# ComparativeGenomicsToolkit/cactus

Hardware: NVIDIA H100
Metric: BAR POA DP Gcells/sec and ends/sec at 1/2/4/8 H100 vs reference CPU BAR (higher is better)
Workload: dtype int32

## Files before the change

cactus_b200/csrc/poa_cta.cuh:

```cuda
#pragma once
#include <cuda_runtime.h>
#include "poa_graph.cuh"
#include "graph_phases.cuh"

namespace barb200 {

__device__ __forceinline__ bool grow_in_par(Graph &g, int t) {
    if (g.in_n[t] < g.in_cap[t]) return true;
    const int ncap = g.in_cap[t] ? g.in_cap[t] * 2 : 2;
    const int noff = atomicAdd(&g.in_used, ncap);
    if (noff + ncap > g.in_pool) { g.err = JOB_ERR_EDGE_CAP; return false; }
    for (int i = 0; i < g.in_n[t]; ++i) { g.in_id[noff + i] = g.in_id[g.in_off[t] + i]; g.in_w[noff + i] = g.in_w[g.in_off[t] + i]; }
    g.in_off[t] = noff; g.in_cap[t] = ncap;
    return true;
}
__device__ __forceinline__ bool grow_out_par(Graph &g, int f) {
    if (g.out_n[f] < g.out_cap[f]) return true;
    const int ncap = g.out_cap[f] ? g.out_cap[f] * 2 : 2;
    const int noff = atomicAdd(&g.out_used, ncap);
    if (noff + ncap > g.out_pool) { g.err = JOB_ERR_EDGE_CAP; return false; }
    const int W = g.W;
    for (int i = 0; i < g.out_n[f]; ++i) {
        g.out_id[noff + i] = g.out_id[g.out_off[f] + i]; g.out_w[noff + i] = g.out_w[g.out_off[f] + i];
        for (int w = 0; w < W; ++w) g.out_rid[(int64_t)(noff + i) * W + w] = g.out_rid[(int64_t)(g.out_off[f] + i) * W + w];
    }
    for (int i = g.out_n[f]; i < ncap; ++i) for (int w = 0; w < W; ++w) g.out_rid[(int64_t)(noff + i) * W + w] = 0;
    g.out_off[f] = noff; g.out_cap[f] = ncap;
    return true;
}
__device__ __forceinline__ void graph_add_edge_par(Graph &g, int from, int to, int check_edge, int read_id) {
    int out_i = -1;
    if (check_edge) {
        const int io = g.in_off[to], in = g.in_n[to];
        for (int i = 0; i < in; ++i) if (g.in_id[io + i] == from) { g.in_w[io + i] += 1; break; }
        const int oo = g.out_off[from], on = g.out_n[from];
        for (int i = 0; i < on; ++i) if (g.out_id[oo + i] == to) { g.out_w[oo + i] += 1; out_i = i; break; }
    }
    if (out_i < 0) {
        if (!grow_in_par(g, to) || !grow_out_par(g, from)) return;
        const int ip = g.in_off[to] + g.in_n[to]; g.in_id[ip] = from; g.in_w[ip] = 1; g.in_n[to]++;
        out_i = g.out_n[from];
        const int op = g.out_off[from] + out_i; g.out_id[op] = to; g.out_w[op] = 1; g.out_n[from]++;
    }
    g.out_rid[(int64_t)(g.out_off[from] + out_i) * g.W + (read_id >> 6)] |= 1ULL << (read_id & 63);
}

__device__ void cta_add_first_sequence(Graph &g, const uint8_t *seq, int len, int read_id) {
    const int tid = threadIdx.x, T = blockDim.x, W = g.W;
    if (len + 2 > g.node_cap) { if (tid == 0) g.err = JOB_ERR_NODE_CAP; __syncthreads(); return; }
    if (2 * (len + 1) > g.in_pool || 2 * (len + 1) > g.out_pool) { if (tid == 0) g.err = JOB_ERR_EDGE_CAP; __syncthreads(); return; }
    const int rw = read_id >> 6; const uint64_t rb = 1ULL << (read_id & 63);
    for (int i = tid; i <= len; i += T) {
        const int to = i < len ? 2 + i : SINK_ID, from = i == 0 ? SRC_ID : 1 + i;
        g.in_off[to] = 2 * i; g.in_n[to] = 1; g.in_cap[to] = 2; g.in_id[2 * i] = from; g.in_w[2 * i] = 1;
        g.out_off[from] = 2 * i; g.out_n[from] = 1; g.out_cap[from] = 2; g.out_id[2 * i] = to; g.out_w[2 * i] = 1;
        for (int w = 0; w < W; ++w) { g.out_rid[(int64_t)(2 * i) * W + w] = w == rw ? rb : 0; g.out_rid[(int64_t)(2 * i + 1) * W + w] = 0; }
        if (i < len) { g.base[to] = seq[i]; g.aln_n[to] = 0; }
        g.index_to_node[i + 1] = to; g.node_to_index[to] = i + 1;
    }
    if (tid == 0) { g.index_to_node[0] = SRC_ID; g.node_to_index[SRC_ID] = 0; }
    if (tid == 0) { g.node_n = len + 2; g.in_used = 2 * (len + 1); g.out_used = 2 * (len + 1); }
    __syncthreads();
}

__device__ void cta_fuse_alignment(Graph &g, const uint8_t *seq, int L, const uint64_t *cigar, int n_cigar, int read_id, int *ws,
                                   unsigned char *scr, int scr_bytes) {
    const int tid = threadIdx.x, T = blockDim.x;
    if (n_cigar == 0) return;
    int *node_of = g.tmp0, *is_new = g.tmp1;
    for (int c = tid; c < n_cigar; c += T) {
        const uint64_t cg = cigar[c];
        const int op = (int)(cg & 0xf);
        if (op == CMATCH) {
            const int node_id = (int)((cg >> 34) & 0x3fffffff), q = (int)((cg >> 4) & 0x3fffffff);
            const uint8_t b = seq[q];
            if (g.base[node_id] == b) { node_of[q] = node_id; is_new[q] = 0; }
            else {
                const int a = graph_aligned_with_base(g, node_id, b);
                if (a != -1) { node_of[q] = a; is_new[q] = 0; } else { node_of[q] = -1 - node_id; is_new[q] = 1; }
            }
        } else if (op == CINS) {
            const int qe = (int)((cg >> 34) & 0x3fffffff), len = (int)((cg >> 4) & 0x3fffffff);
            for (int q = qe - len + 1; q <= qe; ++q) { node_of[q] = INT32_MIN; is_new[q] = 1; }
        }
    }
    __syncthreads();
    const int first_new = g.node_n;
    const int n_new = cta_excl_scan(is_new, L, ws);
    if (first_new + n_new > g.node_cap) { if (tid == 0) g.err = JOB_ERR_NODE_CAP; __syncthreads(); return; }
    for (int q = tid; q < L; q += T) {
        const int m = node_of[q];
        if (m >= 0) { is_new[q] = 0; continue; }
        const int nid = first_new + is_new[q];
        g.base[nid] = seq[q]; g.aln_n[nid] = 0;
        g.in_off[nid] = 0; g.in_n[nid] = 0; g.in_cap[nid] = 0; g.out_off[nid] = 0; g.out_n[nid] = 0; g.out_cap[nid] = 0;
        if (m != INT32_MIN) graph_add_aligned(g, -1 - m, nid);
        node_of[q] = nid; is_new[q] = 1;
    }
    if (tid == 0) g.node_n = first_new + n_new;
    __syncthreads();
    if (g.err) return;
    if (splice_smem_fits(L, first_new, first_new + n_new, scr_bytes)) splice_order_smem(g, node_of, L, first_new, n_new, scr, ws, T);
    else {
        int *anc = g.remain, *cnt = g.msa_rank, *new_i2n = g.tmp1;
        const int n_old = first_new;
        for (int q = tid; q < L; q += T) {
            const int v = node_of[q];
            int e = v < first_new ? g.node_to_index[v] : -1;
            for (int k = 0; k < g.aln_n[v]; ++k) { const int a = g.aln_id[v * 4 + k]; if (a < first_new) e = max(e, g.node_to_index[a]); }
            anc[q] = e;
        }
        for (int i = tid; i < n_old; i += T) cnt[i] = 0;
        __syncthreads();
        cta_incl_max_scan(anc, L, ws);
        for (int q = tid; q < L; q += T) if (node_of[q] >= first_new) atomicAdd(&cnt[max(anc[q], 0)], 1);
        __syncthreads();
        cta_excl_scan(cnt, n_old, ws);
        for (int i = tid; i < n_old; i += T) new_i2n[i + cnt[i]] = g.index_to_node[i];
        for (int q = tid; q < L; q += T) { const int v = node_of[q]; if (v >= first_new) new_i2n[max(anc[q], 0) + 1 + (v - first_new)] = v; }
        __syncthreads();
        for (int k = tid; k < first_new + n_new; k += T) { const int v = new_i2n[k]; g.index_to_node[k] = v; g.node_to_index[v] = k; }
        __syncthreads();
    }
    for (int q = tid; q <= L; q += T) {
        const int from = q == 0 ? SRC_ID : node_of[q - 1], to = q == L ? SINK_ID : node_of[q];
        const int fresh = (q > 0 && from >= first_new) || (q < L && to >= first_new);
        graph_add_edge_par(g, from, to, fresh ? 0 : 1, read_id);
    }
    __syncthreads();
}


__device__ __forceinline__ void prefetch_l2(const void *p) { asm volatile("prefetch.global.L2 [%0];" ::"l"(p)); }

__device__ int warp_backtrack_step(const RowTables &rt, const DpState &d, const PoaParams &P, const int *smat8, const uint8_t *q,
                                   int &i, int &j, int &cur_op, int &len) {
    const unsigned FULLM = 0xffffffffu;
    const int lane = threadIdx.x & 31, inf = P.inf_min, e1 = P.e1, e2 = P.e2, oe1 = P.o1 + P.e1, oe2 = P.o2 + P.e2;
    len = 1;
    const RowRec rc = rt.rec[i];
    const RowInfo ri = d.info[i];
    const int *rowi = d.planes + d.row_off[i];
    const int npre = rc.base_npre >> 8;
    const int s = smat8[8 * (rc.base_npre & 0xff) + q[j - 1]];
    int hij = inf; unsigned cij = (unsigned)E_NEG16 | (unsigned)E_NEG16 << 16;
    if (j >= ri.beg && j <= ri.end) { hij = __ldcg(rowi + plane_index(ri.beg, ri.end, 0, j)); cij = (unsigned)__ldcg(rowi + plane_index(ri.beg, ri.end, 1, j)); }
    int hk0 = inf;
    if ((cur_op & OP_F) && j - 1 - lane >= ri.beg && j - 1 - lane <= ri.end) hk0 = __ldcg(rowi + plane_index(ri.beg, ri.end, 0, j - 1 - lane));
    int pi = -1, pm = inf, ph = inf, pe1 = inf, pe2 = inf; bool m_in = false, e_in = false;
    auto probe = [&](int kb) {
        const int k = kb + lane;
        pi = -1; m_in = false; e_in = false;
        if (k >= npre) return;
        pi = k == 0 ? rc.pre0 : rt.pre_row[rc.pre_off + k];
        const RowInfo pin = d.info[pi];
        const int *prow = d.planes + d.row_off[pi];
        m_in = (cur_op & OP_M) && j - 1 >= pin.beg && j - 1 <= pin.end;
        e_in = (cur_op & OP_E) && j >= pin.beg && j <= pin.end;
        if (m_in) pm = __ldcg(prow + plane_index(pin.beg, pin.end, 0, j - 1));
        if (e_in) {
            ph = __ldcg(prow + plane_index(pin.beg, pin.end, 0, j));
            const unsigned code = (unsigned)__ldcg(prow + plane_index(pin.beg, pin.end, 1, j));
            pe1 = e_decode(ph, (int)(code & 0xffffu), inf); pe2 = e_decode(ph, (int)(code >> 16), inf);
        }
    };
    if (cur_op & OP_M) {
        for (int kb = 0; kb < npre; kb += 32) {
            probe(kb);
            const unsigned hit = __ballot_sync(FULLM, m_in && pm + s == hij);
            if (hit) { i = __shfl_sync(FULLM, pi, __ffs(hit) - 1); --j; cur_op = OP_ALL; return CMATCH; }
        }
    }
    if (cur_op & OP_E) {
        const int own_e1 = e_decode(hij, (int)(cij & 0xffffu), inf), own_e2 = e_decode(hij, (int)(cij >> 16), inf);
        for (int kb = 0; kb < npre; kb += 32) {
            if (npre > 32 || !(cur_op & OP_M)) probe(kb);
            const bool ok1 = e_in && (cur_op & OP_E1) && ((cur_op & OP_M) ? hij == pe1 : own_e1 == pe1 - e1);
            const bool ok2 = e_in && (cur_op & OP_E2) && ((cur_op & OP_M) ? hij == pe2 : own_e2 == pe2 - e2);
            const unsigned hit = __ballot_sync(FULLM, ok1 || ok2);
            if (hit) {
                const int f = __ffs(hit) - 1;
                const int nop = ok1 ? ((ph - oe1 == pe1) ? (OP_M | OP_F) : OP_E1) : ((ph - oe2 == pe2) ? (OP_M | OP_F) : OP_E2);
                cur_op = __shfl_sync(FULLM, nop, f); i = __shfl_sync(FULLM, pi, f);
                return CDEL;
            }
        }
    }
    if (cur_op & OP_F) {
        if (!(cur_op & OP_M)) return -1;
        const int avail = j - ri.beg;
        int t1_max;
        if (e1 > e2) t1_max = oe2 >= oe1 ? (oe2 - oe1) / (e1 - e2) + 1 : 0;
        else t1_max = (e1 < e2 || oe1 <= oe2) ? avail : 0;
        if (t1_max > avail) t1_max = avail;
        for (int which = 0; which < 2; ++which) {
            if (!(cur_op & (which ? OP_F2 : OP_F1))) continue;
            const int oe = which ? oe2 : oe1, e = which ? e2 : e1, tmax = which ? avail : t1_max;
            for (int t0 = 0; t0 < tmax; t0 += 32) {
                const int t = t0 + lane + 1;
                int hk = hk0;
                if (t0 > 0) { hk = inf; if (t <= avail) hk = __ldcg(rowi + plane_index(ri.beg, ri.end, 0, j - t)); }
                const unsigned hit = __ballot_sync(FULLM, t <= tmax && hk == hij + oe + (t - 1) * e);
                if (hit) { len = __ffs(hit); len += t0; j -= len; cur_op = OP_M | OP_E; return CINS; }
            }
        }
    }
    return -1;
}

__device__ void warp_backtrack(Graph &g, const RowTables &rt, DpState &d, const PoaParams &P, const int *smat8, const uint8_t *q, int L) {
    const unsigned FULLM = 0xffffffffu;
    const int lane = threadIdx.x & 31, inf = P.inf_min;
    if (lane == 0) { dp_best_cell(g, rt, d, P, L); d.fc_row = -1; d.fc_hi = -1; }
    __syncwarp();
    int i = d.best_i, j = d.best_j, cur_op = OP_ALL, nc = 0, last_op = -1;
    uint64_t *cg = d.cigar; const int cap = d.cigar_cap;
    int fail = 0;
    auto push = [&](int op, int len, int node_id, int query_id) {
        if (nc == 0 || op != CINS || last_op != CINS) {
            if (nc >= cap) { fail = JOB_ERR_CIGAR_CAP; return; }
            if (lane == 0) {
                const uint64_t n_id = (uint64_t)(int64_t)node_id, q_id = (uint64_t)(int64_t)query_id, l = (uint64_t)len;
                cg[nc] = op == CMATCH ? (n_id << 34 | q_id << 4 | (uint64_t)op) : op == CINS ? (q_id << 34 | l << 4 | (uint64_t)op) : (n_id << 34 | l << 4 | (uint64_t)op);
            }
            ++nc;
        } else if (lane == 0) cg[nc - 1] += (uint64_t)len << 4;
        last_op = op;
    };
    if (j < L) push(CINS, L - j, -1, L - 1);
#ifdef BT_PROFILE
    long long pf_t0 = clock64(), pf_run_t = 0, pf_step_t = 0; int pf_iters = 0, pf_runs = 0, pf_cells = 0, pf_steps = 0, pf_ins = 0;
#endif
    while (i > 0 && j > 0 && !fail) {
        int run = 0;
#ifdef BT_PROFILE
        long long pf_a = clock64();
#endif
        if (cur_op == OP_ALL) {
            int c = i - lane, pre = -1, base = 0, n_ok = 0, node = 0;
            RowInfo ric; ric.beg = 0; ric.end = -1; ric.left = 0; ric.right = 0;
            int64_t ro = 0;
            bool fresh = true;
#pragma unroll 1
            for (int it = 0; it < 4; ++it) {
                if (fresh) {
                    pre = -1;
                    if (c > 0) { const RowRec rc = rt.rec[c]; base = rc.base_npre & 0xff; pre = (rc.base_npre >> 8) ? rc.pre0 : -1; node = g.index_to_node[c]; }
                    if (c >= 0) { ric = d.info[c]; ro = d.row_off[c]; }
                }
                const int nxt = __shfl_down_sync(FULLM, c, 1);
                const bool ok = lane < 31 && pre >= 0 && pre == nxt;
                n_ok = __ffs(~__ballot_sync(FULLM, ok)) - 1;
                if (n_ok >= 31 || it == 3) break;
                const int pre_b = __shfl_sync(FULLM, pre, n_ok);
                if (pre_b < 0) break;
                fresh = lane > n_ok;
                if (fresh) c = pre_b - (lane - n_ok - 1);
            }
            const int jj = j - lane;
            int hv = inf, inb = 0;
            if (lane <= n_ok && c >= 0 && jj >= 0) {
                inb = jj >= ric.beg && jj <= ric.end;
                if (inb) hv = __ldcg(d.planes + ro + plane_index(ric.beg, ric.end, 0, jj));
            }
            const int cl = c - 32, jl = jj - 32;
            RowInfo ril; ril.beg = 0; ril.end = -1; ril.left = 0; ril.right = 0;
            int64_t rol = 0;
            if (cl >= 0 && jl >= 0) { ril = d.info[cl]; rol = d.row_off[cl]; prefetch_l2(rt.rec + cl); prefetch_l2(g.index_to_node + cl); }
            const int h_next = __shfl_down_sync(FULLM, hv, 1), inb_next = __shfl_down_sync(FULLM, inb, 1);
            bool hit = false;
            if (lane < n_ok && c > 0 && jj >= 1 && inb_next) hit = h_next + smat8[8 * base + q[jj - 1]] == hv;
            run = __ffs(~__ballot_sync(FULLM, hit)) - 1;
            if (run > 0) {
                if (nc + run > cap) fail = JOB_ERR_CIGAR_CAP;
                else {
                    if (lane < run) cg[nc + lane] = (uint64_t)node << 34 | (uint64_t)(jj - 1) << 4 | (uint64_t)CMATCH;
                    nc += run; last_op = CMATCH;
                    i = __shfl_sync(FULLM, c, run); j -= run;
                }
            }
            if (cl >= 0 && jl >= 0 && jl <= ril.end) prefetch_l2(d.planes + rol + plane_index(ril.beg, ril.end, 0, jl < ril.beg ? ril.beg : jl));
        }
#ifdef BT_PROFILE
        long long pf_b = clock64(); if (cur_op == OP_ALL) { pf_run_t += pf_b - pf_a; ++pf_iters; if (run) { ++pf_runs; pf_cells += run; } }
#endif
        if (run == 0 && !fail) {
            const int id = g.index_to_node[i], jq = j - 1;
            int len = 1;
            const int op = warp_backtrack_step(rt, d, P, smat8, q, i, j, cur_op, len);
            if (op < 0) fail = JOB_ERR_BACKTRACK; else push(op, len, id, jq);
#ifdef BT_PROFILE
            pf_step_t += clock64() - pf_b; ++pf_steps; if (op == CINS) ++pf_ins;
#endif
        }
    }
#ifdef BT_PROFILE
    if (lane == 0 && blockIdx.x == 0) printf("bt L=%d total=%lld run_t=%lld step_t=%lld iters=%d runs=%d cells=%d steps=%d ins=%d\n", L, clock64() - pf_t0, pf_run_t, pf_step_t, pf_iters, pf_runs, pf_cells, pf_steps, pf_ins);
#endif
    if (!fail && j > 0) push(CINS, j, -1, j - 1);
    if (fail) { if (lane == 0) g.err = fail; return; }
    if (lane == 0) d.n_cigar = nc;
    __syncwarp();
    for (int a = lane; a < nc >> 1; a += 32) { const uint64_t t = cg[a]; cg[a] = cg[nc - 1 - a]; cg[nc - 1 - a] = t; }
    __syncwarp();
}

struct BfsScratch { uint32_t *optr; uint16_t *odst, *queue, *indeg; uint8_t *alnn; };

__device__ __forceinline__ size_t bfs_scratch_bytes(int n, int E) { return (size_t)4 * (n + 1) + (size_t)2 * E + 4 * (size_t)n + n + 16; }

__device__ void bfs_index_smem(Graph &g, const BfsScratch &B) {
    const int n = g.node_n;
    int head = 0, tail = 0;
    B.queue[tail++] = SRC_ID;
    while (head < tail) {
        const int cur = B.queue[head++];
        if (cur == SINK_ID) {
            if (head != n) g.err = JOB_ERR_TOPO;
            return;
        }
        const uint32_t o0 = B.optr[cur], o1 = B.optr[cur + 1];
        for (uint32_t i = o0; i < o1; ++i) {
            const int o = B.odst[i];
            const int left = (int)B.indeg[o] - 1; B.indeg[o] = (uint16_t)left;
            if (left == 0) {
                const int an = B.alnn[o];
                bool ok = true;
                for (int j = 0; j < an; ++j) if (B.indeg[g.aln_id[o * 4 + j]] != 0) { ok = false; break; }
                if (!ok) continue;
                B.queue[tail++] = (uint16_t)o;
                for (int j = 0; j < an; ++j) B.queue[tail++] = (uint16_t)g.aln_id[o * 4 + j];
            }
        }
    }
    g.err = JOB_ERR_TOPO;
}

__device__ void cta_topo_sort(Graph &g, RowTables &rt, unsigned char *scr, int scr_bytes, int *ws, bool have_order) {
    const int tid = threadIdx.x, T = blockDim.x, n = g.node_n;
    if (have_order && topo_smem_fits(n, scr_bytes)) { topo_rows_smem(g, rt, scr, ws, T); return; }
    if (have_order) {
        for (int v = tid; v < n; v += T) graph_sort_node_edges(g, v);
        __syncthreads();
    } else {
    for (int v = tid; v < n; v += T) g.tmp0[v] = g.out_n[v];
    __syncthreads();
    const int E = cta_excl_scan(g.tmp0, n, ws);
    if (n < 65536 && bfs_scratch_bytes(n, E) <= (size_t)scr_bytes) {
        BfsScratch B;
        B.optr = reinterpret_cast<uint32_t *>(scr);
        B.odst = reinterpret_cast<uint16_t *>(B.optr + n + 1);
        B.queue = B.odst + E; B.indeg = B.queue + n;
        B.alnn = reinterpret_cast<uint8_t *>(B.indeg + n);
        for (int v = tid; v < n; v += T) {
            const uint32_t o = (uint32_t)g.tmp0[v];
            B.optr[v] = o;
            const int oo = g.out_off[v], on = g.out_n[v];
            for (int i = 0; i < on; ++i) B.odst[o + i] = (uint16_t)g.out_id[oo + i];
            B.indeg[v] = (uint16_t)g.in_n[v]; B.alnn[v] = g.aln_n[v];
        }
        if (tid == 0) B.optr[n] = (uint32_t)E;
        __syncthreads();
        if (T > 32) {
            if (tid == 0) bfs_index_smem(g, B);
            else if (tid >= 32) for (int v = tid - 32; v < n; v += T - 32) graph_sort_node_edges(g, v);
        } else {
            if (tid == 0) bfs_index_smem(g, B);
            __syncwarp();
            for (int v = tid; v < n; v += T) graph_sort_node_edges(g, v);
        }
        __syncthreads();
        if (g.err) return;
        for (int k = tid; k < n; k += T) { const int v = B.queue[k]; g.index_to_node[k] = v; g.node_to_index[v] = k; }
    } else {
        if (tid == 0) graph_bfs_index(g);
        __syncthreads();
        if (g.err) return;
        for (int v = tid; v < n; v += T) graph_sort_node_edges(g, v);
    }
    __syncthreads();
    }
    int *nx[2] = {g.tmp0, g.tmp1}, *dd[2] = {g.remain, g.msa_rank};
    for (int v = tid; v < n; v += T) {
        int nxt = SINK_ID, dist = 0;
        if (v != SINK_ID) {
            int max_w = -1;
            const int oo = g.out_off[v], on = g.out_n[v];
            for (int i = 0; i < on; ++i) if (g.out_w[oo + i] > max_w) { max_w = g.out_w[oo + i]; nxt = g.out_id[oo + i]; }
            dist = 1;
        }
        nx[0][v] = nxt; dd[0][v] = dist;
    }
    __syncthreads();
    int cur = 0;
    for (int span = 1; span < n; span <<= 1, cur ^= 1) {
        for (int v = tid; v < n; v += T) {
            const int nv = nx[cur][v];
            dd[cur ^ 1][v] = dd[cur][v] + dd[cur][nv];
            nx[cur ^ 1][v] = nx[cur][nv];
        }
        __syncthreads();
    }
    if (cur == 0) { for (int v = tid; v < n; v += T) g.remain[v] -= 1; }
    else { for (int v = tid; v < n; v += T) g.remain[v] = g.msa_rank[v] - 1; }
    __syncthreads();
    for (int r = tid; r < n; r += T) g.tmp0[r] = g.in_n[g.index_to_node[r]];
    __syncthreads();
    cta_excl_scan(g.tmp0, n, ws);
    for (int r = tid; r < n; r += T) graph_build_row(g, rt, r, g.tmp0[r]);
    __syncthreads();
}


__device__ void cta_msa_rank(Graph &g, unsigned char *scr, int scr_bytes, int *ws, int *msa_len_out) {
    const int tid = threadIdx.x, T = blockDim.x, n = g.node_n;
    for (int v = tid; v < n; v += T) g.tmp0[v] = g.out_n[v];
    __syncthreads();
    const int E = cta_excl_scan(g.tmp0, n, ws);
    if (n < 65535 && bfs_scratch_bytes(n, E) + 2 * (size_t)n <= (size_t)scr_bytes) {
        BfsScratch B;
        B.optr = reinterpret_cast<uint32_t *>(scr);
        B.odst = reinterpret_cast<uint16_t *>(B.optr + n + 1);
        B.queue = B.odst + E; B.indeg = B.queue + n;
        uint16_t *rk = B.indeg + n;
        B.alnn = reinterpret_cast<uint8_t *>(rk + n);
        for (int v = tid; v < n; v += T) {
            const uint32_t o = (uint32_t)g.tmp0[v];
            B.optr[v] = o;
            const int oo = g.out_off[v], on = g.out_n[v];
            for (int i = 0; i < on; ++i) B.odst[o + i] = (uint16_t)g.out_id[oo + i];
            B.indeg[v] = (uint16_t)g.in_n[v]; B.alnn[v] = g.aln_n[v];
        }
        if (tid == 0) B.optr[n] = (uint32_t)E;
        __syncthreads();
        if (tid == 0) {
            uint16_t *st = B.queue;
            int sp = 0, rank = 0, len = -1;
            st[sp++] = SRC_ID; rk[SRC_ID] = 0xffff;
            while (sp > 0) {
                const int cur = st[--sp];
                if (rk[cur] == 0xffff) {
                    rk[cur] = (uint16_t)rank;
                    for (int i = 0; i < B.alnn[cur]; ++i) rk[g.aln_id[cur * 4 + i]] = (uint16_t)rank;
                    ++rank;
                }
                if (cur == SINK_ID) { len = (int)rk[SINK_ID] - 1; break; }
                const uint32_t o0 = B.optr[cur], o1 = B.optr[cur + 1];
                for (uint32_t i = o0; i < o1; ++i) {
                    const int o = B.odst[i];
                    const int left = (int)B.indeg[o] - 1; B.indeg[o] = (uint16_t)left;
                    if (left == 0) {
                        const int an = B.alnn[o];
                        bool ok = true;
                        for (int j = 0; j < an; ++j) if (B.indeg[g.aln_id[o * 4 + j]] != 0) { ok = false; break; }
                        if (!ok) continue;
                        st[sp++] = (uint16_t)o; rk[o] = 0xffff;
                        for (int j = 0; j < an; ++j) { const int a = g.aln_id[o * 4 + j]; st[sp++] = (uint16_t)a; rk[a] = 0xffff; }
                    }
                }
            }
            if (len < 0) g.err = JOB_ERR_TOPO;
            *msa_len_out = len;
        }
        __syncthreads();
        if (g.err) return;
        for (int v = tid; v < n; v += T) g.msa_rank[v] = rk[v];
    } else {
        if (tid == 0) *msa_len_out = graph_msa_rank(g);
    }
    __syncthreads();
}

}
```

cactus_b200/csrc/poa_kernel.cu:

```cuda
#include <cuda_runtime.h>
#include <stdint.h>
#include "poa_graph.cuh"
#include "poa_cta.cuh"
#include "poa_kernel.cuh"

namespace barb200 {

#define FULL 0xffffffffu

struct KShared {
    Graph g; RowTables rt; DpState d;
    int job, msa_len_s, abort_s;
    __align__(256) int smat[5 * 8];
    int wF[2][2][32];
    int wM[2][4][32];
    RowRec rec[2];
    RowInfo ring_info[2];
};

__device__ __forceinline__ int4 ld4cg(const int *p) { return __ldcg(reinterpret_cast<const int4 *>(p)); }
__device__ __forceinline__ void st4(int *p, int a, int b, int c, int d) {
    asm volatile("st.global.v4.s32 [%0], {%1, %2, %3, %4};" ::"l"(p), "r"(a), "r"(b), "r"(c), "r"(d) : "memory");
}
__device__ __forceinline__ void sts4(unsigned a, int x, int y, int z, int w) {
    asm volatile("st.shared.v4.s32 [%0], {%1, %2, %3, %4};" ::"r"(a), "r"(x), "r"(y), "r"(z), "r"(w) : "memory");
}
__device__ __forceinline__ int4 lds4(unsigned a) {
    int4 v;
    asm volatile("ld.shared.v4.s32 {%0, %1, %2, %3}, [%4];" : "=r"(v.x), "=r"(v.y), "=r"(v.z), "=r"(v.w) : "r"(a) : "memory");
    return v;
}
__device__ __forceinline__ int lds1(unsigned a) {
    int v;
    asm volatile("ld.shared.s32 %0, [%1];" : "=r"(v) : "r"(a) : "memory");
    return v;
}
__device__ __forceinline__ int lds_const(unsigned a) {
    int v;
    asm("ld.shared.s32 %0, [%1];" : "=r"(v) : "r"(a));
    return v;
}
__device__ __forceinline__ int max3(int a, int b, int c) { return max(max(a, b), c); }
__device__ __forceinline__ void cp_async16(void *smem, const void *gmem) {
    asm volatile("cp.async.cg.shared.global [%0], [%1], 16;" ::"r"((unsigned)__cvta_generic_to_shared(smem)), "l"(gmem) : "memory");
}
__device__ __forceinline__ void cp_async_wait_all() { asm volatile("cp.async.wait_all;" ::: "memory"); }
__device__ __forceinline__ void store_pad(int *tp, int64_t cs, int NEG) {
#pragma unroll
    for (int c = 0; c < TB / CHUNK; ++c) st4(tp + c * cs, c < CPT / CHUNK ? NEG : 0, c < CPT / CHUNK ? NEG : 0, c < CPT / CHUNK ? NEG : 0, c < CPT / CHUNK ? NEG : 0);
}


template <bool MASKED>
__device__ __forceinline__ void row_pass1(int (&H)[CPT], int (&E1)[CPT], int (&E2)[CPT], unsigned mbase, const uint32_t (&qo)[4],
                                          int j0, int beg, int end, int NEG, int e1, int e2, int &agg1, int &agg2) {
#pragma unroll
    for (int e = 0; e < CPT; ++e) {
        const int s = lds_const(__byte_perm(qo[e >> 2], mbase, 0x7650 | (e & 3)));
        int h = __vimax3_s32(H[e] + s, E1[e], E2[e]);
        if (MASKED) {
            const bool inb = (unsigned)(j0 + e - beg) <= (unsigned)(end - beg);
            h = inb ? h : NEG; E1[e] = inb ? E1[e] : NEG; E2[e] = inb ? E2[e] : NEG;
        }
        H[e] = h;
    }
    int a1 = H[CPT - 1], a2 = H[CPT - 1];
#pragma unroll
    for (int e = CPT - 2; e >= 0; --e) { a1 = __viaddmax_s32(a1, e1, H[e]); a2 = __viaddmax_s32(a2, e2, H[e]); }
    agg1 = max(agg1, a1 + j0 * e1); agg2 = max(agg2, a2 + j0 * e2);
}

template <bool ROW0>
__device__ __forceinline__ void pred_chunk(int (&H)[CPT], int (&E1)[CPT], int (&E2)[CPT], int oc, int4 h4, int4 d4, int NEG) {
    const int h[CHUNK] = {h4.x, h4.y, h4.z, h4.w}, dv[CHUNK] = {d4.x, d4.y, d4.z, d4.w};
#pragma unroll
    for (int u = 0; u < CHUNK; ++u) {
        const int e = oc * CHUNK + u;
        const int c1 = dv[u] & 0xffff, c2 = (int)((unsigned)dv[u] >> 16);
        if (e + 1 < CPT) H[e + 1] = max(H[e + 1], h[u]);
        E1[e] = max(E1[e], ROW0 && c1 == E_NEG16 ? NEG : h[u] - c1); E2[e] = max(E2[e], ROW0 && c2 == E_NEG16 ? NEG : h[u] - c2);
    }
}

template <int MODE, int RING_NT>
__device__ __forceinline__ void row_pass2(int (&H)[CPT], int (&E1)[CPT], int (&E2)[CPT], int F1, int F2, int j0, int beg, int end, int NEG,
                                          int e1, int e2, int oe1, int oe2, int *tp, int64_t cs, unsigned rs, int &tmax) {
#pragma unroll
    for (int oc = 0; oc < CPT / CHUNK; ++oc) {
        int dd[CHUNK];
#pragma unroll
        for (int u = 0; u < CHUNK; ++u) {
            const int e = oc * CHUNK + u, hp = H[e];
            int h = __vimax3_s32(hp, F1, F2);
            F1 = __viaddmax_s32(F1, -e1, hp - oe1); F2 = __viaddmax_s32(F2, -e2, hp - oe2);
            int x1 = __viaddmax_s32(E1[e], -e1, h - oe1);
            int x2 = __viaddmax_s32(E2[e], -e2, h - oe2);
            if (MODE == 1) {
                const bool inb = (unsigned)(j0 + e - beg) <= (unsigned)(end - beg);
                h = inb ? h : NEG; x1 = inb ? x1 : NEG; x2 = inb ? x2 : NEG;
            } else if (MODE == 2) {
                const bool inb = j0 + e <= end;
                h = inb ? h : NEG; x1 = inb ? x1 : NEG; x2 = inb ? x2 : NEG;
            }
            H[e] = h; E1[e] = x1; E2[e] = x2;
            dd[u] = __byte_perm(h - x1, h - x2, 0x5410);
            tmax = max(tmax, h);
        }
        st4(tp + oc * cs, H[oc * CHUNK], H[oc * CHUNK + 1], H[oc * CHUNK + 2], H[oc * CHUNK + 3]);
        st4(tp + (CPT / CHUNK + oc) * cs, dd[0], dd[1], dd[2], dd[3]);
        if (RING_NT) {
            sts4(rs + oc * RING_NT * 16, H[oc * CHUNK], H[oc * CHUNK + 1], H[oc * CHUNK + 2], H[oc * CHUNK + 3]);
            sts4(rs + (CPT / CHUNK + oc) * RING_NT * 16, dd[0], dd[1], dd[2], dd[3]);
        }
    }
}

template <bool MASKED>
__device__ __forceinline__ void row_argmax(const int (&H)[CPT], int v, int j0, int beg, int end, int &tl, int &tr) {
    unsigned m = 0;
#pragma unroll
    for (int e = 0; e < CPT; ++e) m |= H[e] == v ? 1u << e : 0u;
    if (MASKED) {
        const int lo = max(beg - j0, 0), hi = min(end - j0, CPT - 1);
        m &= (2u << hi) - (1u << lo);
    }
    if (m) { tl = j0 + __ffs(m) - 1; tr = j0 + 31 - __clz(m); }
}

template <int NT>
__device__ long long dp_sweep(KShared &S, const BatchArgs &A, const uint8_t *__restrict__ qg, int L, uint4 *qsm, unsigned ring) {
    constexpr int RING_NT = poa_ring_bytes(NT) ? NT : 0;
    constexpr unsigned SLOT = NT * TB * sizeof(int), RCS = NT * 16;
    const int tid = threadIdx.x, lane = tid & 31, warp = tid >> 5, nwarps = NT >> 5;
    const unsigned my_ring = ring + tid * 16;
    const PoaParams &P = A.P;
    uint8_t *const sb = A.slots + (int64_t)blockIdx.x * A.lay.slot_bytes;
    const RowRec *const rec_tab = reinterpret_cast<const RowRec *>(sb + A.lay.o_row_rec);
    const int *const pre_row = reinterpret_cast<const int *>(sb + A.lay.o_pre_row);
    RowInfo *const info = reinterpret_cast<RowInfo *>(sb + A.lay.o_row_info);
    int64_t *const row_off = reinterpret_cast<int64_t *>(sb + A.lay.o_row_off);
    int *const planes = A.planes + (int64_t)blockIdx.x * A.lay.plane_cap;
    const int64_t plane_cap = A.lay.plane_cap;
    const int node_n = S.g.node_n, R = node_n - 1;
    const int NEG = P.inf_min, e1 = P.e1, e2 = P.e2, oe1 = P.o1 + P.e1, oe2 = P.o2 + P.e2;
    const int w = P.wb + (int)(P.wf * L);
    const int pn_shift = reference_lane_count(P, L, node_n) == 16 ? 4 : 3;
    static_assert(CPT == 16, "shifts below assume 16 columns per thread");
    const int j0 = tid * CPT;

    uint32_t qo[4] = {0u, 0u, 0u, 0u};
#pragma unroll
    for (int e = 0; e < CPT; ++e) {
        const int j = j0 + e;
        const uint32_t c = (j >= 1 && j <= L) ? qg[j - 1] : 5u;
        qo[e >> 2] |= (4u * c) << ((e & 3) * 8);
    }
    qsm[tid] = make_uint4(qo[0], qo[1], qo[2], qo[3]);
    const unsigned smat_s = (unsigned)__cvta_generic_to_shared(S.smat);

    int H[CPT], E1[CPT], E2[CPT];
    bool prev_active;
    int prev_beg = 0, prev_end, prev_left = 0, prev_right = 0;
    int cur_blk = 0, cells = 0;

    {
        const int dd = L - rec_tab[0].rd;
        prev_end = min(L, max(0, dd) + w);
        const int nT = prev_end / CPT + 1, nTs = row_blocks(0, prev_end);
        if ((int64_t)nTs * TB > plane_cap) return -1;
        prev_active = tid < nT;
        int D[CPT];
#pragma unroll
        for (int e = 0; e < CPT; ++e) {
            const int j = j0 + e;
            if (j == 0) { H[e] = 0; E1[e] = -oe1; E2[e] = -oe2; D[e] = oe1 | (oe2 << 16); }
            else if (j <= prev_end) { H[e] = max(-P.o1 - e1 * j, -P.o2 - e2 * j); E1[e] = NEG; E2[e] = NEG; D[e] = E_NEG16 | (E_NEG16 << 16); }
            else { H[e] = E1[e] = E2[e] = NEG; D[e] = 0; }
        }
        if (tid < nTs) {
            int *tp = planes + chunk_index(nTs, tid, 0);
            const int64_t cs = chunk_index(nTs, 0, 1);
#pragma unroll
            for (int oc = 0; oc < CPT / CHUNK; ++oc) {
                st4(tp + oc * cs, H[oc * CHUNK], H[oc * CHUNK + 1], H[oc * CHUNK + 2], H[oc * CHUNK + 3]);
                st4(tp + (CPT / CHUNK + oc) * cs, D[oc * CHUNK], D[oc * CHUNK + 1], D[oc * CHUNK + 2], D[oc * CHUNK + 3]);
            }
        }
        if (RING_NT) {
#pragma unroll
            for (int oc = 0; oc < CPT / CHUNK; ++oc) {
                sts4(my_ring + oc * RCS, H[oc * CHUNK], H[oc * CHUNK + 1], H[oc * CHUNK + 2], H[oc * CHUNK + 3]);
                sts4(my_ring + (CPT / CHUNK + oc) * RCS, D[oc * CHUNK], D[oc * CHUNK + 1], D[oc * CHUNK + 2], D[oc * CHUNK + 3]);
            }
        }
        if (lane == 31) S.wM[0][3][warp] = H[CPT - 1];
        if (tid == 0) {
            RowInfo ri; ri.beg = 0; ri.end = prev_end; ri.left = 0; ri.right = 0; info[0] = ri; row_off[0] = 0;
            if (RING_NT) S.ring_info[0] = ri;
        }
        cur_blk = nTs; cells = prev_end + 1;
        if (tid == 0) { cp_async16(&S.rec[1], rec_tab + (R > 1 ? 1 : 0)); cp_async_wait_all(); }
    }
    __syncthreads();

    for (int r = 1; r < R; ++r) {
        const int par = r & 1;
        const RowRec rec = S.rec[par];
        if (tid == 0 && r + 1 < R) cp_async16(&S.rec[par ^ 1], rec_tab + r + 1);
        const int b = rec.base_npre & 0xff, npre = rec.base_npre >> 8;
        const int dd = L - rec.rd;
        int maxL = node_n, maxR = 0, min_pre_beg = 0x7fffffff;
        bool has_prev = false;
        if (npre == 1 && rec.pre0 == r - 1) {
            maxL = min(node_n, prev_left + 1); maxR = prev_right + 1; min_pre_beg = prev_beg; has_prev = true;
        } else {
#pragma unroll 1
            for (int k = 0; k < npre; ++k) {
                const int p = k == 0 ? rec.pre0 : pre_row[rec.pre_off + k];
                int pl, pr, pb;
                if (p == r - 1) { pl = prev_left; pr = prev_right; pb = prev_beg; has_prev = true; }
                else if (RING_NT && p == r - 2) { const RowInfo pi = S.ring_info[par]; pl = pi.left; pr = pi.right; pb = pi.beg; }
                else { const RowInfo pi = info[p]; pl = pi.left; pr = pi.right; pb = pi.beg; }
                maxL = min(maxL, pl + 1); maxR = max(maxR, pr + 1); min_pre_beg = min(min_pre_beg, pb);
            }
        }
        const bool only_prev = npre == 1 && has_prev;
        int beg = max(0, min(maxL, dd) - w);
        const int end = min(L, max(maxR, dd) + w);
        if ((beg >> pn_shift) < (min_pre_beg >> pn_shift)) beg = min_pre_beg;
        const int t0 = beg >> 4, nT = (end >> 4) - t0 + 1, tt = tid - t0;
        const int nTs = row_blocks(beg, end), tts = tid - row_t0(beg);
        if ((int64_t)(cur_blk + nTs) * TB > plane_cap) return -1;
        const bool active = tt >= 0 && tt < nT;
        const int wmode = __any_sync(FULL, active && j0 < beg) ? 1 : __any_sync(FULL, active && j0 + CPT - 1 > end) ? 2 : 0;
        const uint32_t qadd = 0x01010101u * (32u * b);

        int hl = __shfl_up_sync(FULL, prev_active ? H[CPT - 1] : NEG, 1);
        if (lane == 0) hl = warp > 0 ? S.wM[par ^ 1][3][warp - 1] : NEG;

        const int id1 = NEG + beg * e1 + P.o1, id2 = NEG + beg * e2 + P.o2;
        int agg1 = id1, agg2 = id2;
        if (active) {
            if (has_prev && prev_active) {
#pragma unroll
                for (int e = CPT - 1; e >= 1; --e) H[e] = H[e - 1];
                H[0] = hl;
            } else {
#pragma unroll
                for (int e = 0; e < CPT; ++e) { H[e] = NEG; E1[e] = NEG; E2[e] = NEG; }
                if (has_prev) H[0] = hl;
            }
#pragma unroll 1
            for (int k = only_prev ? npre : 0; k < npre; ++k) {
                const int p = k == 0 ? rec.pre0 : pre_row[rec.pre_off + k];
                if (p == r - 1) continue;
                if (RING_NT && p == r - 2) {
                    const RowInfo pi = S.ring_info[par];
                    const int pt0 = pi.beg >> 4, pnT = (pi.end >> 4) - pt0 + 1, ptt = tid - pt0;
                    const unsigned rs = my_ring + par * SLOT;
                    if (ptt >= 0 && ptt < pnT) {
                        if (p == 0) {
#pragma unroll
                            for (int oc = 0; oc < CPT / CHUNK; ++oc) pred_chunk<true>(H, E1, E2, oc, lds4(rs + oc * RCS), lds4(rs + (CPT / CHUNK + oc) * RCS), NEG);
                        } else {
#pragma unroll
                            for (int oc = 0; oc < CPT / CHUNK; ++oc) pred_chunk<false>(H, E1, E2, oc, lds4(rs + oc * RCS), lds4(rs + (CPT / CHUNK + oc) * RCS), NEG);
                        }
                    }
                    if (ptt >= 1 && ptt <= pnT) H[0] = max(H[0], lds1(rs + (CPT / CHUNK - 1) * RCS - 4));
                    continue;
                }
                const RowInfo pi = info[p];
                const int pt0 = pi.beg >> 4, pnT = (pi.end >> 4) - pt0 + 1, ptt = tid - pt0, pnTs = row_blocks(pi.beg, pi.end);
                const int *Hp = planes + row_off[p] + chunk_index(pnTs, tid - row_t0(pi.beg), 0);
                const int64_t pcs = chunk_index(pnTs, 0, 1);
                if (ptt >= 0 && ptt < pnT) {
#pragma unroll
                    for (int oc = 0; oc < CPT / CHUNK; ++oc) pred_chunk<true>(H, E1, E2, oc, ld4cg(Hp + oc * pcs), ld4cg(Hp + (CPT / CHUNK + oc) * pcs), NEG);
                }
                if (ptt >= 1 && ptt <= pnT) H[0] = max(H[0], __ldcg(Hp - CHUNK + (CPT / CHUNK - 1) * pcs + CHUNK - 1));
            }
            const uint4 q4 = qsm[tid];
            const uint32_t qo[4] = {q4.x + qadd, q4.y + qadd, q4.z + qadd, q4.w + qadd};
            if (wmode != 1) row_pass1<false>(H, E1, E2, smat_s, qo, j0, beg, end, NEG, e1, e2, agg1, agg2);
            else row_pass1<true>(H, E1, E2, smat_s, qo, j0, beg, end, NEG, e1, e2, agg1, agg2);
        }
        int inc1 = agg1, inc2 = agg2;
#pragma unroll
        for (int off = 1; off < 32; off <<= 1) {
            const int n1 = __shfl_up_sync(FULL, inc1, off), n2 = __shfl_up_sync(FULL, inc2, off);
            if (lane >= off) { inc1 = max(inc1, n1); inc2 = max(inc2, n2); }
        }
        int ex1 = __shfl_up_sync(FULL, inc1, 1), ex2 = __shfl_up_sync(FULL, inc2, 1);
        if (lane == 0) { ex1 = id1; ex2 = id2; }
        if (lane == 31) { S.wF[par][0][warp] = inc1; S.wF[par][1][warp] = inc2; }
        __syncthreads();
        int P1, P2;
        {
            const int wv1 = lane < warp ? S.wF[par][0][lane] : id1, wv2 = lane < warp ? S.wF[par][1][lane] : id2;
            P1 = max(__reduce_max_sync(FULL, wv1), ex1); P2 = max(__reduce_max_sync(FULL, wv2), ex2);
        }
        int tmax = INT32_MIN;
        {
            int *tp = planes + (int64_t)cur_blk * TB + chunk_index(nTs, tts, 0);
            const int64_t cs = chunk_index(nTs, 0, 1);
            const unsigned rs = my_ring + par * SLOT;
            if (active) {
                const int F1 = P1 - P.o1 - j0 * e1, F2 = P2 - P.o2 - j0 * e2;
                if (wmode == 0) row_pass2<0, RING_NT>(H, E1, E2, F1, F2, j0, beg, end, NEG, e1, e2, oe1, oe2, tp, cs, rs, tmax);
                else if (wmode == 2) row_pass2<2, RING_NT>(H, E1, E2, F1, F2, j0, beg, end, NEG, e1, e2, oe1, oe2, tp, cs, rs, tmax);
                else row_pass2<1, RING_NT>(H, E1, E2, F1, F2, j0, beg, end, NEG, e1, e2, oe1, oe2, tp, cs, rs, tmax);
            } else if ((unsigned)tts < (unsigned)nTs) store_pad(tp, cs, NEG);
        }
        {
            const int wmax = __reduce_max_sync(FULL, tmax);
            int tleft = 0x7fffffff, tright = -1;
            if (active && tmax == wmax) {
                if (wmode == 0) row_argmax<false>(H, wmax, j0, beg, end, tleft, tright); else row_argmax<true>(H, wmax, j0, beg, end, tleft, tright);
            }
            const int wl = __reduce_min_sync(FULL, tleft), wr = __reduce_max_sync(FULL, tright);
            if (lane == 0) { S.wM[par][0][warp] = wmax; S.wM[par][1][warp] = wl; S.wM[par][2][warp] = wr; }
            if (lane == 31) S.wM[par][3][warp] = active ? H[CPT - 1] : NEG;
        }
        if (tid == 0) cp_async_wait_all();
        __syncthreads();
        {
            const int v = lane < nwarps ? S.wM[par][0][lane] : INT32_MIN;
            const int bmax = __reduce_max_sync(FULL, v);
            const int l = (lane < nwarps && v == bmax) ? S.wM[par][1][lane] : 0x7fffffff;
            const int rr = (lane < nwarps && v == bmax) ? S.wM[par][2][lane] : -1;
            prev_left = __reduce_min_sync(FULL, l); prev_right = __reduce_max_sync(FULL, rr);
        }
        prev_beg = beg; prev_end = end; prev_active = active;
        if (tid == 0) {
            RowInfo ri; ri.beg = beg; ri.end = end; ri.left = prev_left; ri.right = prev_right; info[r] = ri; row_off[r] = (int64_t)cur_blk * TB;
            if (RING_NT) S.ring_info[par] = ri;
        }
        cur_blk += nTs; cells += end - beg + 1;
    }
    __syncthreads();
    return cells;
}

#define PHASE_TICK(ph) do { if (A.phase_clk && threadIdx.x == 0) { unsigned long long _n = clock64(); A.phase_clk[(size_t)blockIdx.x * PH_N + (ph)] += _n - t_last; t_last = _n; } } while (0)

template <int NT>
__device__ __forceinline__ void poa_msa_body(const BatchArgs &A) {
    extern __shared__ __align__(16) unsigned char dyn_smem[];
    __shared__ KShared S;
    __shared__ uint4 qsm[NT];
    const int tid = threadIdx.x;
    int *ws = &S.wF[0][0][0];
    if (tid == 0) { const int slot = blockIdx.x; slot_views(A.lay, A.slots + (int64_t)slot * A.lay.slot_bytes, A.planes + (int64_t)slot * A.lay.plane_cap, S.g, S.rt, S.d); }
    for (int k = tid; k < 40; k += blockDim.x) S.smat[k] = (k & 7) < 5 ? A.P.mat[(k >> 3) * 5 + (k & 7)] : 0;
    unsigned long long t_last = A.phase_clk ? clock64() : 0ULL, t_start = t_last;
    __syncthreads();

    while (true) {
        if (tid == 0) {
            const int k = atomicAdd(A.next_job, 1);
            int j = -1;
            if (k < A.n_jobs) j = A.job_base + k;
            S.job = j;
        }
        __syncthreads();
        const int job = S.job;
        if (job < 0) break;
        const JobDesc jd = A.jobs[job];
        const int K = jd.n_seq;
        const int *lens = A.lens + jd.len_off;
        const int64_t *soff = A.soff + jd.len_off;
        const uint8_t *seqs = A.seqs + jd.seq_off;
        if (tid == 0) { graph_reset(S.g, K); S.abort_s = 0; }
        __syncthreads();
        const int *const order = A.order + jd.len_off;
        if (tid == 0 && A.gt_status[job]) S.g.err = JOB_ERR_GT_CAP;
        __syncthreads();
        long long cells = 0;
        for (int a = 0; a < K && !S.g.err; ++a) {
            const int read = order[a], L = lens[read];
            const uint8_t *q = seqs + soff[read];
            if (a == 0) {
                if (A.serial_phases) { if (tid == 0) graph_add_first_sequence(S.g, q, L, read); }
                else cta_add_first_sequence(S.g, q, L, read);
                PHASE_TICK(PH_FUSE);
            } else {
                long long c = -2;
                if (L + 1 <= CPT * (int)blockDim.x) c = dp_sweep<NT>(S, A, q, L, qsm, (unsigned)__cvta_generic_to_shared(dyn_smem));
                if (c < 0) { if (tid == 0) S.g.err = c == -2 ? JOB_ERR_QUERY_LEN : JOB_ERR_PLANE_CAP; c = 0; }
                cells += c;
                __syncthreads();
                PHASE_TICK(PH_DP);
                if (A.serial_phases) { if (tid == 0 && !S.g.err) { dp_best_cell(S.g, S.rt, S.d, A.P, L); dp_backtrack(S.g, S.rt, S.d, A.P, q, L); } }
                else if (tid < 32 && !S.g.err) warp_backtrack(S.g, S.rt, S.d, A.P, S.smat, q, L);
                PHASE_TICK(PH_BACKTRACK);
                __syncthreads();
                if (A.serial_phases) { if (tid == 0 && !S.g.err) graph_fuse_alignment(S.g, q, S.d.cigar, S.d.n_cigar, read); }
                else if (!S.g.err) cta_fuse_alignment(S.g, q, L, S.d.cigar, S.d.n_cigar, read, ws, dyn_smem, A.scratch_bytes);
                PHASE_TICK(PH_FUSE);
            }
            __syncthreads();
            if (S.g.err) break;
            if (A.serial_phases) { if (tid == 0) graph_topo_sort_serial(S.g, S.rt); __syncthreads(); }
            else cta_topo_sort(S.g, S.rt, dyn_smem, A.scratch_bytes, ws, A.bfs_order == 0);
            PHASE_TICK(PH_TOPO);
            if (S.g.err) break;
        }
        __syncthreads();
        if (!S.g.err) {
            if (A.serial_phases) { if (tid == 0) S.msa_len_s = graph_msa_rank(S.g); __syncthreads(); }
            else cta_msa_rank(S.g, dyn_smem, A.scratch_bytes, ws, &S.msa_len_s);
            if (tid == 0 && !S.g.err && S.msa_len_s > jd.msa_stride) S.g.err = JOB_ERR_MSA_CAP;
        }
        __syncthreads();
        if (!S.g.err) {
            const int ml = S.msa_len_s;
            uint8_t *msa = A.msa + jd.msa_off;
            for (int64_t i = tid; i < (int64_t)K * ml; i += blockDim.x) msa[(i / ml) * jd.msa_stride + (i % ml)] = GAP_CODE;
            __syncthreads();
            for (int v = 2 + tid; v < S.g.node_n; v += blockDim.x) graph_msa_fill_node(S.g, v, msa, jd.msa_stride);
        }
        __syncthreads();
        if (tid == 0) { A.status[job] = S.g.err; A.msa_len[job] = S.g.err ? 0 : S.msa_len_s; A.cells[job] = cells; }
        PHASE_TICK(PH_MSA);
        __syncthreads();
    }
    if (A.phase_clk && tid == 0) A.phase_clk[(size_t)blockIdx.x * PH_N + PH_TOTAL] += clock64() - t_start;
}

extern "C" __global__ void __launch_bounds__(32, 16) poa_msa_kernel_t32(const BatchArgs A) { poa_msa_body<32>(A); }
extern "C" __global__ void __launch_bounds__(64, 8) poa_msa_kernel_t64(const BatchArgs A) { poa_msa_body<64>(A); }
#ifndef BARB200_T128_MINB
#define BARB200_T128_MINB 4
#endif
extern "C" __global__ void __launch_bounds__(128, BARB200_T128_MINB) poa_msa_kernel_t128(const BatchArgs A) { poa_msa_body<128>(A); }
extern "C" __global__ void __launch_bounds__(256, 2) poa_msa_kernel_t256(const BatchArgs A) { poa_msa_body<256>(A); }
extern "C" __global__ void __launch_bounds__(640, 1) poa_msa_kernel_t640(const BatchArgs A) { poa_msa_body<640>(A); }
extern "C" __global__ void __launch_bounds__(1024, 1) poa_msa_kernel_t1024(const BatchArgs A) { poa_msa_body<1024>(A); }

}
```

Measured before the change: 263.6.

## Stage backtrack row metadata in a shared-memory sliding window via cp.async

```diff
diff --git a/cactus_b200/csrc/bt_window.cuh b/cactus_b200/csrc/bt_window.cuh
--- /dev/null
+++ b/cactus_b200/csrc/bt_window.cuh
@@ -0,0 +1,103 @@
+#pragma once
+#include "poa_types.h"
+
+namespace barb200 {
+
+constexpr int BT_ROW_BYTES = 36;
+constexpr int BT_MIN_ROWS = 64;
+constexpr int BT_LAND_MARGIN = 64;
+
+struct BtWindow {
+    unsigned base;
+    int cap;
+    int lo, hi;
+    int plo;
+#ifdef BT_PROFILE
+    int refills, fallbacks;
+#endif
+};
+
+struct BtRow {
+    RowRec rec;
+    int beg, end;
+    int64_t off;
+    int node;
+};
+
+__device__ __forceinline__ BtWindow bt_window(unsigned char *scr, int scr_bytes) {
+    BtWindow w;
+    w.base = (unsigned)__cvta_generic_to_shared(scr);
+    const int rows = scr_bytes / BT_ROW_BYTES;
+    w.cap = rows < BT_MIN_ROWS ? 0 : 1 << (31 - __clz(rows));
+    w.lo = 0; w.hi = -1; w.plo = 0;
+#ifdef BT_PROFILE
+    w.refills = 0; w.fallbacks = 0;
+#endif
+    return w;
+}
+
+__device__ __forceinline__ void bt_cp16(unsigned s, const void *g) { asm volatile("cp.async.cg.shared.global [%0], [%1], 16;" ::"r"(s), "l"(g) : "memory"); }
+__device__ __forceinline__ void bt_cp8(unsigned s, const void *g) { asm volatile("cp.async.ca.shared.global [%0], [%1], 8;" ::"r"(s), "l"(g) : "memory"); }
+__device__ __forceinline__ void bt_cp4(unsigned s, const void *g) { asm volatile("cp.async.ca.shared.global [%0], [%1], 4;" ::"r"(s), "l"(g) : "memory"); }
+
+__device__ __forceinline__ void bt_fill(const BtWindow &w, const Graph &g, const RowTables &rt, const DpState &d, int a, int b) {
+    const unsigned C = (unsigned)w.cap;
+    for (int r = a + (int)(threadIdx.x & 31); r <= b; r += 32) {
+        const unsigned s = (unsigned)r & (C - 1);
+        bt_cp16(w.base + 16 * s, rt.rec + r);
+        bt_cp8(w.base + 16 * C + 8 * s, d.info + r);
+        bt_cp8(w.base + 24 * C + 8 * s, d.row_off + r);
+        bt_cp4(w.base + 32 * C + 4 * s, g.index_to_node + r);
+    }
+}
+
+__device__ __forceinline__ void bt_land(BtWindow &w) {
+    asm volatile("cp.async.wait_all;" ::: "memory");
+    __syncwarp();
+    w.lo = w.plo;
+}
+
+__device__ __forceinline__ void bt_advance(BtWindow &w, const Graph &g, const RowTables &rt, const DpState &d, int i) {
+    if (w.plo < w.lo) {
+        if (i >= w.lo + BT_LAND_MARGIN) return;
+        bt_land(w);
+    }
+    const int half = w.cap >> 1;
+    if (w.lo == 0 || i >= w.lo + half) return;
+    if (i >= w.lo) {
+        w.hi = imin(w.hi, w.lo + half - 1);
+        w.plo = imax(0, w.lo - half);
+        bt_fill(w, g, rt, d, w.plo, w.lo - 1);
+    } else {
+        w.hi = i; w.lo = i + 1;
+        w.plo = imax(0, i - w.cap + 1);
+        bt_fill(w, g, rt, d, w.plo, i);
+    }
+#ifdef BT_PROFILE
+    ++w.refills;
+#endif
+}
+
+__device__ __forceinline__ BtRow bt_row(BtWindow &w, const Graph &g, const RowTables &rt, const DpState &d, int r) {
+    BtRow x;
+    if (r >= w.lo && r <= w.hi) {
+        const unsigned C = (unsigned)w.cap, s = (unsigned)r & (C - 1);
+        asm volatile("ld.shared.v4.s32 {%0, %1, %2, %3}, [%4];"
+                     : "=r"(x.rec.base_npre), "=r"(x.rec.rd), "=r"(x.rec.pre_off), "=r"(x.rec.pre0) : "r"(w.base + 16 * s));
+        asm volatile("ld.shared.v2.s32 {%0, %1}, [%2];" : "=r"(x.beg), "=r"(x.end) : "r"(w.base + 16 * C + 8 * s));
+        asm volatile("ld.shared.s64 %0, [%1];" : "=l"(x.off) : "r"(w.base + 24 * C + 8 * s));
+        asm volatile("ld.shared.s32 %0, [%1];" : "=r"(x.node) : "r"(w.base + 32 * C + 4 * s));
+    } else {
+        x.rec = rt.rec[r];
+        const RowInfo ri = d.info[r];
+        x.beg = ri.beg; x.end = ri.end;
+        x.off = d.row_off[r];
+        x.node = g.index_to_node[r];
+#ifdef BT_PROFILE
+        ++w.fallbacks;
+#endif
+    }
+    return x;
+}
+
+}
diff --git a/cactus_b200/csrc/poa_cta.cuh b/cactus_b200/csrc/poa_cta.cuh
--- a/cactus_b200/csrc/poa_cta.cuh
+++ b/cactus_b200/csrc/poa_cta.cuh
@@ -2,6 +2,7 @@
 #include <cuda_runtime.h>
 #include "poa_graph.cuh"
 #include "graph_phases.cuh"
+#include "bt_window.cuh"
 
 namespace barb200 {
 
@@ -133,14 +134,13 @@
 
 __device__ __forceinline__ void prefetch_l2(const void *p) { asm volatile("prefetch.global.L2 [%0];" ::"l"(p)); }
 
-__device__ int warp_backtrack_step(const RowTables &rt, const DpState &d, const PoaParams &P, const int *smat8, const uint8_t *q,
-                                   int &i, int &j, int &cur_op, int &len) {
+__device__ __forceinline__ int warp_backtrack_step(BtWindow &w, const Graph &g, const RowTables &rt, const DpState &d, const PoaParams &P,
+                                                   const int *smat8, const uint8_t *q, const BtRow &ri, int &i, int &j, int &cur_op, int &len) {
     const unsigned FULLM = 0xffffffffu;
     const int lane = threadIdx.x & 31, inf = P.inf_min, e1 = P.e1, e2 = P.e2, oe1 = P.o1 + P.e1, oe2 = P.o2 + P.e2;
     len = 1;
-    const RowRec rc = rt.rec[i];
-    const RowInfo ri = d.info[i];
-    const int *rowi = d.planes + d.row_off[i];
+    const RowRec rc = ri.rec;
+    const int *rowi = d.planes + ri.off;
     const int npre = rc.base_npre >> 8;
     const int s = smat8[8 * (rc.base_npre & 0xff) + q[j - 1]];
     int hij = inf; unsigned cij = (unsigned)E_NEG16 | (unsigned)E_NEG16 << 16;
@@ -153,8 +153,8 @@
         pi = -1; m_in = false; e_in = false;
         if (k >= npre) return;
         pi = k == 0 ? rc.pre0 : rt.pre_row[rc.pre_off + k];
-        const RowInfo pin = d.info[pi];
-        const int *prow = d.planes + d.row_off[pi];
+        const BtRow pin = bt_row(w, g, rt, d, pi);
+        const int *prow = d.planes + pin.off;
         m_in = (cur_op & OP_M) && j - 1 >= pin.beg && j - 1 <= pin.end;
         e_in = (cur_op & OP_E) && j >= pin.beg && j <= pin.end;
         if (m_in) pm = __ldcg(prow + plane_index(pin.beg, pin.end, 0, j - 1));
@@ -208,11 +208,14 @@
     return -1;
 }
 
-__device__ void warp_backtrack(Graph &g, const RowTables &rt, DpState &d, const PoaParams &P, const int *smat8, const uint8_t *q, int L) {
+__device__ __noinline__ void warp_backtrack(Graph &g, const RowTables &rt, DpState &d, const PoaParams P, const int *smat8, const uint8_t *q, int L,
+                                            unsigned char *scr, int scr_bytes) {
     const unsigned FULLM = 0xffffffffu;
     const int lane = threadIdx.x & 31, inf = P.inf_min;
+    BtWindow w = bt_window(scr, scr_bytes);
+    if (w.cap) { w.hi = g.node_n - 1; w.lo = g.node_n; w.plo = imax(0, g.node_n - w.cap); bt_fill(w, g, rt, d, w.plo, w.hi); }
     if (lane == 0) { dp_best_cell(g, rt, d, P, L); d.fc_row = -1; d.fc_hi = -1; }
-    __syncwarp();
+    bt_land(w);
     int i = d.best_i, j = d.best_j, cur_op = OP_ALL, nc = 0, last_op = -1;
     uint64_t *cg = d.cigar; const int cap = d.cigar_cap;
     int fail = 0;
@@ -233,20 +236,23 @@
 #endif
     while (i > 0 && j > 0 && !fail) {
         int run = 0;
+        if (w.cap) bt_advance(w, g, rt, d, i);
 #ifdef BT_PROFILE
         long long pf_a = clock64();
 #endif
         if (cur_op == OP_ALL) {
-            int c = i - lane, pre = -1, base = 0, n_ok = 0, node = 0;
-            RowInfo ric; ric.beg = 0; ric.end = -1; ric.left = 0; ric.right = 0;
+            int c = i - lane, pre = -1, base = 0, n_ok = 0, node = 0, beg = 0, end = -1;
             int64_t ro = 0;
             bool fresh = true;
 #pragma unroll 1
             for (int it = 0; it < 4; ++it) {
                 if (fresh) {
                     pre = -1;
-                    if (c > 0) { const RowRec rc = rt.rec[c]; base = rc.base_npre & 0xff; pre = (rc.base_npre >> 8) ? rc.pre0 : -1; node = g.index_to_node[c]; }
-                    if (c >= 0) { ric = d.info[c]; ro = d.row_off[c]; }
+                    if (c >= 0) {
+                        const BtRow x = bt_row(w, g, rt, d, c);
+                        beg = x.beg; end = x.end; ro = x.off;
+                        if (c > 0) { base = x.rec.base_npre & 0xff; pre = (x.rec.base_npre >> 8) ? x.rec.pre0 : -1; node = x.node; }
+                    }
                 }
                 const int nxt = __shfl_down_sync(FULLM, c, 1);
                 const bool ok = lane < 31 && pre >= 0 && pre == nxt;
@@ -260,13 +266,13 @@
             const int jj = j - lane;
             int hv = inf, inb = 0;
             if (lane <= n_ok && c >= 0 && jj >= 0) {
-                inb = jj >= ric.beg && jj <= ric.end;
-                if (inb) hv = __ldcg(d.planes + ro + plane_index(ric.beg, ric.end, 0, jj));
+                inb = jj >= beg && jj <= end;
+                if (inb) hv = __ldcg(d.planes + ro + plane_index(beg, end, 0, jj));
             }
             const int cl = c - 32, jl = jj - 32;
-            RowInfo ril; ril.beg = 0; ril.end = -1; ril.left = 0; ril.right = 0;
+            int lbeg = 0, lend = -1;
             int64_t rol = 0;
-            if (cl >= 0 && jl >= 0) { ril = d.info[cl]; rol = d.row_off[cl]; prefetch_l2(rt.rec + cl); prefetch_l2(g.index_to_node + cl); }
+            if (cl >= 0 && jl >= 0) { const BtRow x = bt_row(w, g, rt, d, cl); lbeg = x.beg; lend = x.end; rol = x.off; }
             const int h_next = __shfl_down_sync(FULLM, hv, 1), inb_next = __shfl_down_sync(FULLM, inb, 1);
             bool hit = false;
             if (lane < n_ok && c > 0 && jj >= 1 && inb_next) hit = h_next + smat8[8 * base + q[jj - 1]] == hv;
@@ -279,23 +285,28 @@
                     i = __shfl_sync(FULLM, c, run); j -= run;
                 }
             }
-            if (cl >= 0 && jl >= 0 && jl <= ril.end) prefetch_l2(d.planes + rol + plane_index(ril.beg, ril.end, 0, jl < ril.beg ? ril.beg : jl));
+            if (cl >= 0 && jl >= 0 && jl <= lend) prefetch_l2(d.planes + rol + plane_index(lbeg, lend, 0, jl < lbeg ? lbeg : jl));
         }
 #ifdef BT_PROFILE
         long long pf_b = clock64(); if (cur_op == OP_ALL) { pf_run_t += pf_b - pf_a; ++pf_iters; if (run) { ++pf_runs; pf_cells += run; } }
 #endif
         if (run == 0 && !fail) {
-            const int id = g.index_to_node[i], jq = j - 1;
+            const BtRow ri = bt_row(w, g, rt, d, i);
+            const int jq = j - 1;
             int len = 1;
-            const int op = warp_backtrack_step(rt, d, P, smat8, q, i, j, cur_op, len);
-            if (op < 0) fail = JOB_ERR_BACKTRACK; else push(op, len, id, jq);
+            const int op = warp_backtrack_step(w, g, rt, d, P, smat8, q, ri, i, j, cur_op, len);
+            if (op < 0) fail = JOB_ERR_BACKTRACK; else push(op, len, ri.node, jq);
 #ifdef BT_PROFILE
             pf_step_t += clock64() - pf_b; ++pf_steps; if (op == CINS) ++pf_ins;
 #endif
         }
     }
+    bt_land(w);
 #ifdef BT_PROFILE
-    if (lane == 0 && blockIdx.x == 0) printf("bt L=%d total=%lld run_t=%lld step_t=%lld iters=%d runs=%d cells=%d steps=%d ins=%d\n", L, clock64() - pf_t0, pf_run_t, pf_step_t, pf_iters, pf_runs, pf_cells, pf_steps, pf_ins);
+    const int pf_fb = __reduce_add_sync(FULLM, w.fallbacks);
+    if (lane == 0 && blockIdx.x == 0)
+        printf("bt L=%d total=%lld run_t=%lld step_t=%lld iters=%d runs=%d cells=%d steps=%d ins=%d window=%d refills=%d fallbacks=%d\n", L,
+               clock64() - pf_t0, pf_run_t, pf_step_t, pf_iters, pf_runs, pf_cells, pf_steps, pf_ins, w.cap, w.refills, pf_fb);
 #endif
     if (!fail && j > 0) push(CINS, j, -1, j - 1);
     if (fail) { if (lane == 0) g.err = fail; return; }
diff --git a/cactus_b200/csrc/poa_kernel.cu b/cactus_b200/csrc/poa_kernel.cu
--- a/cactus_b200/csrc/poa_kernel.cu
+++ b/cactus_b200/csrc/poa_kernel.cu
@@ -392,7 +392,7 @@
                 __syncthreads();
                 PHASE_TICK(PH_DP);
                 if (A.serial_phases) { if (tid == 0 && !S.g.err) { dp_best_cell(S.g, S.rt, S.d, A.P, L); dp_backtrack(S.g, S.rt, S.d, A.P, q, L); } }
-                else if (tid < 32 && !S.g.err) warp_backtrack(S.g, S.rt, S.d, A.P, S.smat, q, L);
+                else if (tid < 32 && !S.g.err) warp_backtrack(S.g, S.rt, S.d, A.P, S.smat, q, L, dyn_smem, A.scratch_bytes);
                 PHASE_TICK(PH_BACKTRACK);
                 __syncthreads();
                 if (A.serial_phases) { if (tid == 0 && !S.g.err) graph_fuse_alignment(S.g, q, S.d.cigar, S.d.n_cigar, read); }
```

After: 270.5 (median of 6 runs). 2.6% higher.
